# MiloniAtal/gato-python

Measured on AMD Instinct MI355X. Metric: PCG iterations/s, higher is better.
Workload: dtype f64; 1 GPU; iiwa_14_7_k50_f64; STATE_SIZE=14, CONTROL_SIZE=7, KNOT_POINTS=50, max_iters=100, pcg_kernel=resident (one workgroup, mixed 2/1 rows per lane), pcg_workgroups=1, pcg_threads=512

## Files before the change

### gato_python_amd/csrc/gato_assembly.hip

```cpp
#include "gato_common.h"
#include "gato_gj.h"

namespace gato {
namespace {

constexpr int WAVE = 64;

template <typename T, int S, int C>
__global__ void add_rho_kernel(const T *__restrict__ G_in, T rho, T *__restrict__ Gd, size_t n_per_sys, int B)
{
    constexpr int SS = S * S, CC = C * C;
    const size_t total = n_per_sys * B;
    for (size_t i = (size_t)blockIdx.x * blockDim.x + threadIdx.x; i < total; i += (size_t)gridDim.x * blockDim.x) {
        const size_t w = (i % n_per_sys) % (SS + CC);
        const bool diag = w < SS ? (w % (S + 1) == 0) : ((w - SS) % (C + 1) == 0);
        Gd[i] = G_in[i] + (diag ? rho : (T)0);
    }
}

__device__ __forceinline__ void wave_sync() { __syncthreads(); }

template <typename T>
__device__ __forceinline__ void copy_in(T *dst, const T *__restrict__ src, int n, int lane)
{
// ... 221 lines not shown
        Pbd[i] = diag ? (T)1 / Sbd[i] : (T)0;
    }
}

template <typename T, int S>
__global__ __launch_bounds__(WAVE) void ss_kernel(const T *__restrict__ Sbd, T *__restrict__ Pbd, int K, BatchStride bs)
{
    constexpr int SS = S * S;
    int sysi, kidx;
    xcd_knot_map(sysi, kidx);
    Sbd += sysi * bs.bd; Pbd += sysi * bs.bd;
    constexpr bool STAGE = S > 16;
    __shared__ T sT[2][SS];
    __shared__ T stage[STAGE ? 5 * SS : 1];
    const int lane = threadIdx.x;
    for (int k = bs.k_lo + kidx; k < bs.k_hi; k += gridDim.x) {
        T *Pk = Pbd + (size_t)k * 3 * SS;
        const T *sPm = Pk + SS;
        const bool has_l = k > 0, has_r = k < K - 1;
        const T *xl = Sbd + (size_t)k * 3 * SS, *xr = Sbd + (size_t)(k + 1) * 3 * SS;
        const T *pl = Pbd + (size_t)(k - 1) * 3 * SS + SS, *pr = Pbd + (size_t)(k + 1) * 3 * SS + SS;
        wave_sync();
        if constexpr (STAGE) {
            copy_in(stage, sPm, SS, lane);
            if (has_l) { copy_in(stage + SS, xl, SS, lane); copy_in(stage + 2 * SS, pl, SS, lane); }
            if (has_r) { copy_in(stage + 3 * SS, xr, SS, lane); copy_in(stage + 4 * SS, pr, SS, lane); }
            sPm = stage; xl = stage + SS; pl = stage + 2 * SS; xr = stage + 3 * SS; pr = stage + 4 * SS;
            wave_sync();
        }
        if (has_l) {
            const T *sX = xl;
            mfma_for_tiles<T, S, S>(lane,
                [&](int mt, int nt, typename Mfma<T>::acc_t acc) { return mfma_tile<T, S, S, S, false>(sPm, sX, mt, nt, lane, acc); },
                [&](int r, int cc, T v) { sT[0][cc * S + r] = v; });
        }
        if (has_r) {
            const T *sX = xr;
            mfma_for_tiles<T, S, S>(lane,
                [&](int mt, int nt, typename Mfma<T>::acc_t acc) { return mfma_tile<T, S, S, S, true>(sPm, sX, mt, nt, lane, acc); },
                [&](int r, int cc, T v) { sT[1][cc * S + r] = v; });
        }
        wave_sync();
        if (has_l) {
            const T *sPn = pl;
            mfma_for_tiles<T, S, S>(lane,
                [&](int mt, int nt, typename Mfma<T>::acc_t acc) { return mfma_tile<T, S, S, S, false>(sT[0], sPn, mt, nt, lane, acc); },
                [&](int r, int cc, T v) { Pk[cc * S + r] = -v; });
        }
        if (has_r) {
            const T *sPn = pr;
            mfma_for_tiles<T, S, S>(lane,
                [&](int mt, int nt, typename Mfma<T>::acc_t acc) { return mfma_tile<T, S, S, S, false>(sT[1], sPn, mt, nt, lane, acc); },
                [&](int r, int cc, T v) { Pk[2 * SS + cc * S + r] = -v; });
        }
    }
}

template <int NT, typename T>
__device__ __forceinline__ void copy_nt(T *dst, const T *__restrict__ src, int n, int tid)
{
    for (int i = tid; i < n; i += NT) dst[i] = src[i];
}

template <typename T, int M, int N, int NW, typename TileFn, typename StoreFn>
__device__ __forceinline__ void mfma_tiles_on_waves(int wave, int lane, int first, TileFn tile, StoreFn store)
{
    constexpr int NTN = (N + 15) / 16;
#pragma unroll
    for (int mt = 0; mt < (M + 15) / 16; ++mt) {
#pragma unroll
        for (int nt = 0; nt < NTN; ++nt) {
            if ((first + mt * NTN + nt) % NW != wave) continue;
            typename Mfma<T>::acc_t acc = {0, 0, 0, 0};
            acc = tile(mt, nt, acc);
#pragma unroll
            for (int j = 0; j < 4; ++j) {
                const int r = mt * 16 + Mfma<T>::row(lane, j), c = nt * 16 + (lane & 15);
                if (r < M && c < N) store(r, c, acc[j]);
            }
        }
    }
}

template <typename T, int S, int C>
struct AsmLds {
    static constexpr int n = S + C, SS = S * S, CC = C * C, SC = S * C;
    static constexpr int Q = 0;
    static constexpr int R = Q + 3 * SS;
    static constexpr int AB = R + 3 * CC;
    static constexpr int PHI = AB + 2 * (SS + SC);
    static constexpr int BR = PHI + 2 * SS;
    static constexpr int TH = BR + 2 * SC;
    static constexpr int TT = TH + 2 * SS;
    static constexpr int VQ = TT + 2 * SS;
    static constexpr int VV = VQ + 2 * S + C;
    static constexpr int ELEMS = (VV + 3 * S + 3) / 4 * 4;
    static constexpr int PTR_G = 3 * n + 1, PTR_C = 2 * S + 1;
    static constexpr size_t BYTES = sizeof(T) * ELEMS + sizeof(int) * (PTR_G + PTR_C);
};

__device__ __forceinline__ int row_of_entry(const int *ptr, int nrows, int e)
{
    int lo = 0, hi = nrows;
    while (hi - lo > 1) {
        const int mid = (lo + hi) >> 1;
        if (ptr[mid] <= e) lo = mid; else hi = mid;
    }
    return lo;
}

template <typename T, int S, int C, int NT>
__global__ __launch_bounds__(NT, (GatherWaves<T, S>::v)) void gather_kernel(const int *__restrict__ G_row, const int *__restrict__ G_col,
                                                    const T *__restrict__ G_val, const int *__restrict__ C_row,
                                                    const int *__restrict__ C_col, const T *__restrict__ C_val, int K, T rho,
                                                    T *__restrict__ Gd, T *__restrict__ Cd, T *__restrict__ Ginv, BatchStride bs)
{
    constexpr int n = S + C, SS = S * S, CC = C * C, SC = S * C, ABS = SS + SC;
    static_assert(NT % WAVE == 0, "whole waves");
    __shared__ T blk[SS + CC + ABS];
    __shared__ int sPtrG[n + 1], sPtrC[S + 1];
    constexpr int NSLOT = SS + CC + ABS;
    __shared__ unsigned smask[(NSLOT + 31) / 32];
    __shared__ int sown[NSLOT];
    __shared__ int s_coll;
    T *sQ = blk, *sR = blk + SS, *sAB = blk + SS + CC;
    const int tid = threadIdx.x, lane = tid & 63, wave = tid >> 6;
    G_val += blockIdx.y * bs.nnzG; C_val += blockIdx.y * bs.nnzC;
    Gd += blockIdx.y * bs.g; Cd += blockIdx.y * bs.c;
    if (Ginv) Ginv += blockIdx.y * bs.g;
    for (int k = bs.k_lo + blockIdx.x; k < bs.k_hi; k += gridDim.x) {
        const bool last = k == K - 1;
        const int r0 = k * n, nrG = last ? S : n;
        const int c0 = (k + 1) * S, nrC = last ? 0 : S;
        __syncthreads();
        for (int i = tid; i <= nrG; i += NT) sPtrG[i] = G_row[r0 + i];
        if (nrC) for (int i = tid; i <= nrC; i += NT) sPtrC[i] = C_row[c0 + i];
        for (int i = tid; i < SS + CC + ABS; i += NT) blk[i] = (T)0;
        for (int i = tid; i < (NSLOT + 31) / 32; i += NT) smask[i] = 0u;
        if (tid == 0) s_coll = 0;
        __syncthreads();
        const int eG0 = sPtrG[0], nG = sPtrG[nrG] - eG0;
        const int eC0 = nrC ? sPtrC[0] : 0, nC = nrC ? sPtrC[nrC] - eC0 : 0;
        auto slot_of = [&](int t, int colv, T valv, T &v) -> int {
            if (t < nG) {
                const int isr = row_of_entry(sPtrG, nrG, eG0 + t);
                const int isc = colv % n;
                v = valv + (colv == r0 + isr ? rho : (T)0);
                if (isc < S) return isr < S ? isc * S + isr : -1;
                return isr >= S ? SS + (isc - S) * C + (isr - S) : -1;
            }
            const int i = row_of_entry(sPtrC, nrC, eC0 + (t - nG));
            v = valv;
            return colv / n <= k ? SS + CC + (colv % n) * S + i : -1;
        };
        constexpr int U = 4;
        for (int t0 = tid; t0 < nG + nC; t0 += NT * U) {
            int col[U];
            T val[U];
#pragma unroll
            for (int u = 0; u < U; ++u) {
                const int t = t0 + u * NT;
                if (t < nG) { col[u] = G_col[eG0 + t]; val[u] = G_val[eG0 + t]; }
                else if (t < nG + nC) { col[u] = C_col[eC0 + (t - nG)]; val[u] = C_val[eC0 + (t - nG)]; }
            }
#pragma unroll
            for (int u = 0; u < U; ++u) {
                const int t = t0 + u * NT;
                if (t < nG + nC) {
                    T v;
                    const int sl = slot_of(t, col[u], val[u], v);
                    if (sl >= 0) {
                        blk[sl] = v;
                        const unsigned bit = 1u << (sl & 31);
                        if (atomicOr(&smask[sl >> 5], bit) & bit) s_coll = 1;
                    }
                }
            }
        }
        __syncthreads();
        if (s_coll) {
            for (int i = tid; i < NSLOT; i += NT) sown[i] = -1;
            __syncthreads();
            for (int pass = 0; pass < 2; ++pass) {
                for (int t = tid; t < nG + nC; t += NT) {
                    const int colv = t < nG ? G_col[eG0 + t] : C_col[eC0 + (t - nG)];
                    const T valv = t < nG ? G_val[eG0 + t] : C_val[eC0 + (t - nG)];
                    T v;
                    const int sl = slot_of(t, colv, valv, v);
                    if (sl < 0) continue;
                    if (pass == 0) atomicMax(&sown[sl], t);
                    else if (sown[sl] == t) blk[sl] = v;
                }
                __syncthreads();
            }
        }
        __syncthreads();
        const size_t gk = (size_t)k * (SS + CC);
        for (int i = tid; i < SS + (last ? 0 : CC); i += NT) Gd[gk + i] = blk[i];
        if (!last) for (int i = tid; i < ABS; i += NT) Cd[(size_t)k * ABS + i] = sAB[i];
        if (Ginv) {
            if (wave == 0) invert_to<T, S>(sQ, Ginv + gk, lane, (T)1);
            if (wave == (NT > WAVE ? 1 : 0) && !last) invert_to<T, C>(sR, Ginv + gk + SS, lane, (T)1);
        }
    }
}

template <typename T, int S, int C, int NT>
__global__ __launch_bounds__(NT) void assemble_kernel(AsmArgs a, int K, BatchStride bs)
{
    typedef AsmLds<T, S, C> L;
    constexpr int n = S + C, SS = S * S, CC = C * C, SC = S * C, NW = NT / WAVE, ABS = SS + SC;
    static_assert(NW >= 6, "six inversions run side by side");
    constexpr int TILES = ((S + 15) / 16) * ((S + 15) / 16);
    extern __shared__ __align__(16) unsigned char lds_raw[];
    T *lds = (T *)lds_raw;
    T *sQ = lds + L::Q, *sR = lds + L::R, *sAB = lds + L::AB, *sPhi = lds + L::PHI, *sBR = lds + L::BR;
    T *sTh = lds + L::TH, *sT = lds + L::TT, *sq = lds + L::VQ, *sv = lds + L::VV;
    int *sPtrG = (int *)(lds + L::ELEMS), *sPtrC = sPtrG + L::PTR_G;
    constexpr int NSLOT = 3 * SS + 3 * CC + 2 * ABS;
    __shared__ unsigned smask[(NSLOT + 31) / 32];
    __shared__ int sown[NSLOT];
    __shared__ int s_coll;
    const int tid = threadIdx.x, lane = tid & 63, wave = tid >> 6;
    const int sys = blockIdx.y;
    const T *g = (const T *)a.g + sys * bs.n, *c = (const T *)a.c + sys * bs.sk;
    T *Gd = (T *)a.Gd + sys * bs.g, *Cd = (T *)a.Cd + sys * bs.c, *Ginv = (T *)a.Ginv + sys * bs.g;
    T *Sbd = (T *)a.Sbd + sys * bs.bd, *Pbd = (T *)a.Pbd + sys * bs.bd, *gamma = (T *)a.gamma + sys * bs.sk;
    const T rho = (T)a.rho;
    T *const iS = (T *)a.imgS, *const iP = (T *)a.imgP;
    const size_t ild = (size_t)a.img_ld;
    auto imS = [&](int kk, int b, int r, int cc, T v) { if (iS) iS[(size_t)(b * S + cc) * ild + (size_t)kk * S + r] = v; };
    auto imP = [&](int kk, int b, int r, int cc, T v) { if (iP) iP[(size_t)(b * S + cc) * ild + (size_t)kk * S + r] = v; };
    T *sQk = sQ + 2 * SS, *sRk = sR + 2 * CC, *sQm = sQ + SS, *sRm = sR + CC, *sQmm = sQ, *sRmm = sR;
    T *sA1 = sAB + ABS, *sB1 = sA1 + SS, *sA0 = sAB, *sB0 = sAB + SS;
    T *sPhi1 = sPhi + SS, *sPhi0 = sPhi, *sBR1 = sBR + SC, *sBR0 = sBR, *sTh1 = sTh + SS, *sTh0 = sTh;
    int n_stamp = 0;
    auto stamp = [&]() {
        if (a.stamps && blockIdx.x == (K > 2 ? 2 : 0) && sys == 0 && tid == 0) a.stamps[n_stamp++] = __builtin_amdgcn_s_memrealtime();
    };
    stamp();

    for (int k = blockIdx.x; k < K; k += gridDim.x) {
        const bool first = k == 0, last = k == K - 1;
        const bool full0 = k >= 2;
        const size_t gk = (size_t)k * (SS + CC);
        const size_t cm = first ? 0 : (size_t)(k - 1) * ABS;
        T *Sk = Sbd + (size_t)k * 3 * SS, *Pk = Pbd + (size_t)k * 3 * SS;
        __syncthreads();
        if (a.mode == 0) {
            const T *G_val = (const T *)a.G_val + sys * bs.nnzG, *C_val = (const T *)a.C_val + sys * bs.nnzC;
            const int r0 = (k >= 2 ? k - 2 : 0) * n, nrG = k * n + (last ? S : n) - r0;
            const int c0 = (k >= 2 ? k - 1 : 1) * S, nrC = first ? 0 : (k + 1) * S - c0;
            for (int i = tid; i <= nrG; i += NT) sPtrG[i] = a.G_row[r0 + i];
            if (nrC) for (int i = tid; i <= nrC; i += NT) sPtrC[i] = a.C_row[c0 + i];
            for (int i = tid; i < 3 * SS + 3 * CC + 2 * ABS; i += NT) lds[i] = (T)0;
            for (int i = tid; i < (NSLOT + 31) / 32; i += NT) smask[i] = 0u;
            if (tid == 0) s_coll = 0;
            __syncthreads();
            const int eG0 = sPtrG[0], nG = sPtrG[nrG] - eG0;
            const int eC0 = nrC ? sPtrC[0] : 0, nC = nrC ? sPtrC[nrC] - eC0 : 0;
            auto slot_of = [&](int t, int colv, T valv, T &v) -> int {
                if (t < nG) {
                    const int row = r0 + row_of_entry(sPtrG, nrG, eG0 + t);
                    const int knot = row / n, isr = row - knot * n, qi = knot - (k - 2);
                    const int isc = colv % n;
                    v = valv + (colv == row ? rho : (T)0);
                    if (isc < S) return isr < S ? L::Q + qi * SS + isc * S + isr : -1;
                    return isr >= S ? L::R + qi * CC + (isc - S) * C + (isr - S) : -1;
                }
                const int row = c0 + row_of_entry(sPtrC, nrC, eC0 + (t - nG));
                const int br = row / S - 1, i = row - (br + 1) * S;
                v = valv;
                return colv / n <= br ? L::AB + (br - (k - 2)) * ABS + (colv % n) * S + i : -1;
            };
            constexpr int U = 4;
            for (int t0 = tid; t0 < nG + nC; t0 += NT * U) {
                int col[U];
                T val[U];
#pragma unroll
                for (int u = 0; u < U; ++u) {
                    const int t = t0 + u * NT;
                    if (t < nG) { col[u] = a.G_col[eG0 + t]; val[u] = G_val[eG0 + t]; }
                    else if (t < nG + nC) { col[u] = a.C_col[eC0 + (t - nG)]; val[u] = C_val[eC0 + (t - nG)]; }
                }
#pragma unroll
                for (int u = 0; u < U; ++u) {
                    const int t = t0 + u * NT;
                    if (t < nG + nC) {
                        T v;
                        const int sl = slot_of(t, col[u], val[u], v);
                        if (sl >= 0) {
                            lds[sl] = v;
                            const unsigned bit = 1u << (sl & 31);
                            if (atomicOr(&smask[sl >> 5], bit) & bit) s_coll = 1;
                        }
                    }
                }
            }
            __syncthreads();
            if (s_coll) {
                for (int i = tid; i < NSLOT; i += NT) sown[i] = -1;
                __syncthreads();
                for (int pass = 0; pass < 2; ++pass) {
                    for (int t = tid; t < nG + nC; t += NT) {
                        const int colv = t < nG ? a.G_col[eG0 + t] : a.C_col[eC0 + (t - nG)];
                        const T valv = t < nG ? G_val[eG0 + t] : C_val[eC0 + (t - nG)];
                        T v;
                        const int sl = slot_of(t, colv, valv, v);
                        if (sl < 0) continue;
                        if (pass == 0) atomicMax(&sown[sl], t);
                        else if (sown[sl] == t) lds[sl] = v;
                    }
                    __syncthreads();
                }
            }
        } else {
            const T *Gin = a.mode == 2 ? (const T *)a.G_val + sys * bs.g : Gd;
            const T r2 = a.mode == 2 ? rho : (T)0;
#pragma unroll
            for (int qi = 0; qi < 3; ++qi) {
                const int knot = k - 2 + qi;
                if (knot < 0) continue;
                const size_t go = (size_t)knot * (SS + CC);
                for (int i = tid; i < SS; i += NT) sQ[qi * SS + i] = Gin[go + i] + ((i % (S + 1) == 0) ? r2 : (T)0);
                if (knot < K - 1)
                    for (int i = tid; i < CC; i += NT) sR[qi * CC + i] = Gin[go + SS + i] + ((i % (C + 1) == 0) ? r2 : (T)0);
                if (qi < 2 && knot < K - 1) copy_nt<NT>(sAB + qi * ABS, Cd + (size_t)knot * ABS, ABS, tid);
            }
        }
        if (first) { for (int i = tid; i < S; i += NT) sq[i] = g[i]; }
        else {
            copy_nt<NT>(sq, g + (size_t)(k - 1) * n, n, tid);
            for (int i = tid; i < S; i += NT) sq[n + i] = g[(size_t)k * n + i];
        }
        __syncthreads();
        stamp();
        if (a.mode != 1) {
            for (int i = tid; i < SS; i += NT) Gd[gk + i] = sQk[i];
            if (!last) for (int i = tid; i < CC; i += NT) Gd[gk + SS + i] = sRk[i];
            if (a.mode == 0 && !first) for (int i = tid; i < ABS; i += NT) Cd[cm + i] = sA1[i];
        }
        if (first) for (int i = tid; i < SS; i += NT) { Pk[SS + i] = -sQk[i]; imP(0, 1, i % S, i / S, -sQk[i]); }
        if (k == 1) for (int i = tid; i < SS; i += NT) sTh0[i] = -sQm[i];
        __syncthreads();
        if (wave == 0) invert_to<T, S>(sQk, sQk, lane, (T)1);
        else if (wave == 1) { if (!first) invert_to<T, S>(sQm, sQm, lane, (T)1); }
        else if (wave == 2) { if (!first) invert_to<T, C>(sRm, sRm, lane, (T)1); }
        else if (wave == 3) { if (full0) invert_to<T, S>(sQmm, sQmm, lane, (T)1); }
        else if (wave == 4) { if (full0) invert_to<T, C>(sRmm, sRmm, lane, (T)1); }
        else if (wave == 5) { if (!last) invert_to<T, C>(sRk, sRk, lane, (T)1); }
        __syncthreads();
        stamp();
        for (int i = tid; i < SS; i += NT) Ginv[gk + i] = sQk[i];
        if (!last) for (int i = tid; i < CC; i += NT) Ginv[gk + SS + i] = sRk[i];
        if (first) {
            if (wave == 0) mv<T, S, S>(sv, sQk, sq, lane);
            for (int i = tid; i < SS; i += NT) {
                Sk[i] = (T)0;
                Sk[SS + i] = -sQk[i];
                Pk[i] = (T)0;
                if (last) { Pk[2 * SS + i] = (T)0; Sk[2 * SS + i] = (T)0; }
                imS(0, 0, i % S, i / S, (T)0); imS(0, 1, i % S, i / S, -sQk[i]); imP(0, 0, i % S, i / S, (T)0);
                if (last) { imP(0, 2, i % S, i / S, (T)0); imS(0, 2, i % S, i / S, (T)0); }
            }
            __syncthreads();
            for (int i = tid; i < S; i += NT) gamma[i] = c[i] - sv[i];
            continue;
        }
        mfma_tiles_on_waves<T, S, S, NW>(wave, lane, 0,
            [&](int mt, int nt, typename Mfma<T>::acc_t acc) { return mfma_tile<T, S, S, S, false>(sA1, sQm, mt, nt, lane, acc); },
            [&](int r, int cc, T v) {
                sPhi1[cc * S + r] = v;
                Sk[cc * S + r] = -v;
                Sk[2 * SS - 3 * SS + r * S + cc] = -v;
                imS(k, 0, r, cc, -v); imS(k - 1, 2, cc, r, -v);
            });
        mfma_tiles_on_waves<T, S, C, NW>(wave, lane, TILES,
            [&](int mt, int nt, typename Mfma<T>::acc_t acc) { return mfma_tile<T, S, C, C, false>(sB1, sRm, mt, nt, lane, acc); },
            [&](int r, int cc, T v) { sBR1[cc * S + r] = v; });
        if (full0) {
            mfma_tiles_on_waves<T, S, S, NW>(wave, lane, 2 * TILES,
                [&](int mt, int nt, typename Mfma<T>::acc_t acc) { return mfma_tile<T, S, S, S, false>(sA0, sQmm, mt, nt, lane, acc); },
                [&](int r, int cc, T v) { sPhi0[cc * S + r] = v; });
            mfma_tiles_on_waves<T, S, C, NW>(wave, lane, 3 * TILES,
                [&](int mt, int nt, typename Mfma<T>::acc_t acc) { return mfma_tile<T, S, C, C, false>(sB0, sRmm, mt, nt, lane, acc); },
                [&](int r, int cc, T v) { sBR0[cc * S + r] = v; });
        }
        if (wave == NW - 1) mv<T, S, S>(sv, sQk, sq + n, lane);
        __syncthreads();
        if (wave == NW - 1) mv<T, S, S>(sv + S, sPhi1, sq, lane);
        if (wave == NW - 2) mv<T, S, C>(sv + 2 * S, sBR1, sq + S, lane);
        mfma_tiles_on_waves<T, S, S, NW>(wave, lane, 0,
            [&](int mt, int nt, typename Mfma<T>::acc_t acc) {
                acc = mfma_tile<T, S, S, S, true>(sPhi1, sA1, mt, nt, lane, acc);
                return mfma_tile<T, S, C, S, true>(sBR1, sB1, mt, nt, lane, acc);
            },
            [&](int r, int cc, T v) {
                const T th = v + sQk[cc * S + r];
                sTh1[cc * S + r] = th;
                Sk[SS + cc * S + r] = -th;
                imS(k, 1, r, cc, -th);
            });
        if (full0)
            mfma_tiles_on_waves<T, S, S, NW>(wave, lane, TILES,
                [&](int mt, int nt, typename Mfma<T>::acc_t acc) {
                    acc = mfma_tile<T, S, S, S, true>(sPhi0, sA0, mt, nt, lane, acc);
                    return mfma_tile<T, S, C, S, true>(sBR0, sB0, mt, nt, lane, acc);
                },
                [&](int r, int cc, T v) { sTh0[cc * S + r] = v + sQm[cc * S + r]; });
        __syncthreads();
        if (wave == 0) invert_to<T, S>(sTh1, sTh1, lane, (T)-1);
        else if (wave == 1) { if (full0) invert_to<T, S>(sTh0, sTh0, lane, (T)-1); }
        else {
            for (int i = tid - 2 * WAVE; i < S; i += NT - 2 * WAVE) {
                T gt = sv[i] - c[(size_t)k * S + i];
                gt += sv[2 * S + i] + sv[S + i];
                gamma[(size_t)k * S + i] = -gt;
            }
            if (last)
                for (int i = tid - 2 * WAVE; i < SS; i += NT - 2 * WAVE) {
                    Pk[2 * SS + i] = (T)0;
                    Sk[2 * SS + i] = (T)0;
                    imP(k, 2, i % S, i / S, (T)0); imS(k, 2, i % S, i / S, (T)0);
                }
        }
        __syncthreads();
        stamp();
        for (int i = tid; i < SS; i += NT) { Pk[SS + i] = sTh1[i]; imP(k, 1, i % S, i / S, sTh1[i]); }
        mfma_tiles_on_waves<T, S, S, NW>(wave, lane, 0,
            [&](int mt, int nt, typename Mfma<T>::acc_t acc) { return mfma_tile<T, S, S, S, false>(sTh1, sPhi1, mt, nt, lane, acc); },
            [&](int r, int cc, T v) { sT[cc * S + r] = v; });
        mfma_tiles_on_waves<T, S, S, NW>(wave, lane, TILES,
            [&](int mt, int nt, typename Mfma<T>::acc_t acc) { return mfma_tile<T, S, S, S, true>(sTh0, sPhi1, mt, nt, lane, acc); },
            [&](int r, int cc, T v) { sT[SS + cc * S + r] = v; });
        __syncthreads();
        mfma_tiles_on_waves<T, S, S, NW>(wave, lane, 0,
            [&](int mt, int nt, typename Mfma<T>::acc_t acc) { return mfma_tile<T, S, S, S, false>(sT, sTh0, mt, nt, lane, acc); },
            [&](int r, int cc, T v) { Pk[cc * S + r] = v; imP(k, 0, r, cc, v); });
        mfma_tiles_on_waves<T, S, S, NW>(wave, lane, TILES,
            [&](int mt, int nt, typename Mfma<T>::acc_t acc) { return mfma_tile<T, S, S, S, false>(sT + SS, sTh1, mt, nt, lane, acc); },
            [&](int r, int cc, T v) { Pk[2 * SS - 3 * SS + cc * S + r] = v; imP(k - 1, 2, r, cc, v); });
        stamp();
    }
}


template <typename T, int S, int C>
__global__ __launch_bounds__(WAVE) void dz_kernel(const T *__restrict__ Ginv, const T *__restrict__ Cd,
                                                  const T *__restrict__ g, const T *__restrict__ lambda,
                                                  int K, T *__restrict__ dz, BatchStride bs)
{
    constexpr int n = S + C, SS = S * S, CC = C * C, SC = S * C;
    int sysi, kidx;
    xcd_knot_map(sysi, kidx);
    const int msys = bs.rhs > 1 ? sysi / bs.rhs : sysi;
    Ginv += msys * bs.g; Cd += msys * bs.c; g += sysi * bs.n; lambda += sysi * bs.sk;
    dz += sysi * bs.n;
    __shared__ T sQi[SS], sA[SS], sRi[CC > 0 ? CC : 1], sB[SC > 0 ? SC : 1], sl[2 * S], st[S + C], sg[S + C];
    const int lane = threadIdx.x;
    for (int k = bs.k_lo + kidx; k < bs.k_hi; k += gridDim.x) {
        const bool last = k == K - 1;
        wave_sync();
        copy_in(sQi, Ginv + (size_t)k * (SS + CC), SS, lane);
        copy_in(sl, lambda + (size_t)k * S, last ? S : 2 * S, lane);
        copy_in(sg, g + (size_t)k * n, last ? S : n, lane);
        if (!last) {
            copy_in(sRi, Ginv + (size_t)k * (SS + CC) + SS, CC, lane);
            copy_in(sA, Cd + (size_t)k * (SS + SC), SS, lane);
            copy_in(sB, Cd + (size_t)k * (SS + SC) + SS, SC, lane);
        }
        wave_sync();
        if (!last) {
            mTv<T, S, S>(st, sA, sl + S, lane);
            mTv<T, S, C>(st + S, sB, sl + S, lane);
            wave_sync();
            for (int i = lane; i < S; i += WAVE) st[i] = sg[i] - (sl[i] + st[i]);
            for (int i = lane; i < C; i += WAVE) st[S + i] = sg[S + i] - st[S + i];
        } else {
            for (int i = lane; i < S; i += WAVE) st[i] = sg[i] - sl[i];
        }
        wave_sync();
        for (int r = lane; r < S; r += WAVE) {
            T res = (T)0;
#pragma unroll
            for (int cc = 0; cc < S; ++cc) res = gato::fmaT(sQi[r + cc * S], st[cc], res);
            dz[(size_t)k * n + r] = res;
        }
        if (!last) {
            for (int r = lane; r < C; r += WAVE) {
                T res = (T)0;
#pragma unroll
                for (int cc = 0; cc < C; ++cc) res = gato::fmaT(sRi[r + cc * C], st[S + cc], res);
                dz[(size_t)k * n + S + r] = res;
            }
        }
    }
}

}

template <typename T, int S, int C>
int launch_convert(const Dims &d, const int *G_row, const int *G_col, const T *G_val, const int *C_row,
                   const int *C_col, const T *C_val, T rho, T *Gd, T *Cd, T *Ginv, hipStream_t st)
{
    constexpr int NT = S <= 16 ? 64 : 128;
    hipLaunchKernelGGL((gather_kernel<T, S, C, NT>), dim3(d.hi() - d.lo() < (1 << 20) ? d.hi() - d.lo() : (1 << 20), d.B), dim3(NT), 0, st, G_row, G_col,
                       G_val, C_row, C_col, C_val, d.K, rho, Gd, Cd, Ginv, batch_stride(d));
    GATO_HIP_CHECK(hipGetLastError());
    return GATO_OK;
}

template <typename T, int S, int C>
int launch_add_rho(const Dims &d, const T *G_in, T rho, T *Gd, hipStream_t st)
{
    const size_t total = d.g_dense() * d.B;
    const int blocks = (int)((total + 255) / 256 < 2048 ? (total + 255) / 256 : 2048);
    hipLaunchKernelGGL((add_rho_kernel<T, S, C>), dim3(blocks), dim3(256), 0, st, G_in, rho, Gd, d.g_dense(), d.B);
    GATO_HIP_CHECK(hipGetLastError());
    return GATO_OK;
}

static inline int knot_grid(int K) { return K < 8192 ? K : 8192; }

template <typename T, int S, int C>
int launch_form_schur(const Dims &d, const T *Gd, const T *Cd, const T *g, const T *c, T *Sbd, T *Pbd,
// ... 93 lines not shown
```

### gato_python_amd/csrc/gato_capi.hip

```cpp
#include <cmath>
#include <cstdarg>
#include <cstdlib>
#include "gato_solver.h"

namespace gato {

static thread_local char g_err[512] = "";

void set_error(const char *fmt, ...)
{
    va_list ap;
    va_start(ap, fmt);
    vsnprintf(g_err, sizeof(g_err), fmt, ap);
    va_end(ap);
}

}

using namespace gato;

bool solver_usable(const gato_solver *s, const char *entry, const char *unsupported)
{
    if (!s) set_error("%s: null solver", entry);
    else if (s->cl.on || s->cl.local) set_error("%s: the solver is a cluster rank; sharded %s are not supported", entry, unsupported);
// ... 139 lines not shown
    const size_t o_S = take(d.bd() * e * nb), o_P = take(d.bd() * e * nb), o_gam = take(d.sk() * e * nb);
    const size_t o_lam = take(d.sk() * e * nb), o_dz = take(d.N() * e * nb);
    const size_t o_its = take(sizeof(int) * nb);
    const size_t o_vec = take(6 * d.sk() * e);
    const size_t o_part = take((size_t)4 * max_groups * e), o_scal = take(64 * 8), o_done = take(64);
    const size_t o_gh = take((size_t)8 * S * e);
    const size_t o_hist = take(sizeof(double) * (GATO_ETA_HIST_MAX + 1));
    const size_t o_xtab = take(sizeof(void *) * GATO_MAX_RANKS);
    const long long rows = (long long)K * S;
    const bool img = B == 1 && ((s->plan.pair_threads > 0 && rows <= 2ll * s->plan.pair_threads) || (s->plan.mixed_rows > 0 && rows <= s->plan.mixed_rows));
    int img_ld = 0;
    if (img) {
        img_ld = (int)((rows + 63) / 64 * 64) + 128;
        if (img_ld < s->plan.mixed_rows) img_ld = s->plan.mixed_rows;
    }
    const size_t o_iS = take(img ? (size_t)3 * S * img_ld * e : 0), o_iP = take(img ? (size_t)3 * S * img_ld * e : 0);
    s->arena_bytes = off;
    GATO_HIP_CHECK(hipMalloc((void **)&s->arena, off));
    GATO_HIP_CHECK(hipMemset(s->arena, 0, off));
    char *a = s->arena;
    s->slots = (unsigned long long *)(a + o_slots);
    s->status = (int *)(a + o_status);
    s->iters = B > 1 ? (int *)(a + o_its) : (int *)(a + o_status + 8);
    s->final_eta = (double *)(a + o_status + 16);
    s->tune_status = (int *)(a + o_status + 32); s->tune_iters = (int *)(a + o_status + 40); s->tune_eta = (double *)(a + o_status + 48);
    s->dz_flag = (int *)(a + o_status + 56);
    s->G_dense = a + o_G; s->C_dense = a + o_C; s->Ginv = a + o_Gi;
    s->Sbd = a + o_S; s->Pbd = a + o_P; s->gamma = a + o_gam; s->lambda = a + o_lam; s->dz = a + o_dz;
    s->sw.vecs = a + o_vec;
    s->sw.partials = a + o_part; s->sw.scalars = a + o_scal; s->sw.done = (int *)(a + o_done);
    s->sw.max_groups = max_groups;
    s->ghosts = a + o_gh;
    s->eta_hist = (double *)(a + o_hist);
    s->cl_tab = (unsigned long long **)(a + o_xtab);
    if (img) { s->imgS = a + o_iS; s->imgP = a + o_iP; s->img_ld = img_ld; }
    const char *nt = getenv("GATO_NO_TUNE");
    if (!(nt && atoi(nt))) {
        const int rc = gato_solver_tune(s, nullptr);
        if (rc) { gato_solver_destroy(s); return rc; }
    }
    *out = s;
    return GATO_OK;
}

extern "C" int gato_solver_destroy(gato_solver *s)
{
    if (!s) return GATO_OK;
    (void)hipSetDevice(s->device);
    gato_cluster_destroy(s);
    if (s->ev_pcg0) (void)hipEventDestroy(s->ev_pcg0);
    if (s->ev_pcg1) (void)hipEventDestroy(s->ev_pcg1);
    if (s->ev_cal0) (void)hipEventDestroy(s->ev_cal0);
    if (s->ev_cal1) (void)hipEventDestroy(s->ev_cal1);
    for (int i = 0; i < 4; ++i)
        if (s->ev_stage[i]) (void)hipEventDestroy(s->ev_stage[i]);
    if (s->arena) (void)hipFree(s->arena);
    if (s->rhs_ws) (void)hipFree(s->rhs_ws);
    if (s->qp_ws) (void)hipFree(s->qp_ws);
    if (s->pol_ws) (void)hipFree(s->pol_ws);
    if (s->in_arena) (void)hipFree(s->in_arena);
    for (int i = 0; i < 2; ++i)
        if (s->host_ev[i]) (void)hipEventDestroy(s->host_ev[i]);
    if (s->pin) (void)hipHostFree(s->pin);
    delete s;
    return GATO_OK;
}

extern "C" void *gato_solver_buffer(gato_solver *s, int which)
{
    switch (which) {
        case 0: return s->G_dense;
        case 1: return s->C_dense;
        case 2: return s->Ginv;
        case 3: return s->Sbd;
        case 4: return s->Pbd;
        case 5: return s->gamma;
        case 6: return s->lambda;
        case 7: return s->dz;
        case 8: return s->iters;
        case 9: return (unsigned long long *)s->sw.scalars + 8;
        case 10: return s->eta_hist;
        case 11: return s->rhs_ws;
        case 12: return s->qp_pcg_total;
        default: return nullptr;
    }
}

extern "C" int gato_solver_set_option(gato_solver *s, const char *name, int value)
{
    if (!strcmp(name, "pcg_mode")) s->pcg_mode = value;
    else if (!strcmp(name, "pcg_threads")) s->pcg_threads = value;
    else if (!strcmp(name, "pcg_groups")) s->pcg_groups = value;
    else if (!strcmp(name, "asm_mode")) s->asm_mode = value;
    else if (!strcmp(name, "pcg_semi")) s->pcg_semi = value;
    else if (!strcmp(name, "pcg_epoch")) s->pcg_epoch = (unsigned)value;
    else if (!strcmp(name, "cluster_epoch")) s->cl.xepoch = (unsigned)value;
    else if (!strcmp(name, "stamp_asm")) s->stamp_asm = value;
    else if (!strcmp(name, "stamp_pcg")) s->stamp_pcg = value;
    else if (!strcmp(name, "ablate")) s->ablate = value;
    else if (!strcmp(name, "no_single_lds")) s->no_single_lds = value;
    else if (!strcmp(name, "no_pair")) s->no_pair = value;
    else if (!strcmp(name, "wave_pub")) s->wave_pub = value;
    else if (!strcmp(name, "dpp_rows")) s->dpp_rows = value;
    else if (!strcmp(name, "pcg_variant")) s->pcg_variant = value;
    else if (!strcmp(name, "record_eta")) s->record_eta = value;
    else if (!strcmp(name, "xcd_pack")) s->xcd_pack = value;
    else if (!strcmp(name, "xcd_sel")) s->xcd_sel = value < 0 ? -1 : (value & 7);
    else if (!strcmp(name, "true_warm_start")) s->true_warm_start = value;
    else if (!strcmp(name, "timeout_ms")) s->timeout_ms = value > 0 ? value : 2000;
    else if (!strcmp(name, "max_workgroups")) s->max_workgroups = value;
    else if (!strcmp(name, "no_fuse_dz")) s->no_fuse_dz = value;
    else if (!strcmp(name, "no_image")) s->no_image = value;
    else if (!strcmp(name, "coop_launch")) s->coop_launch = value;
    else if (!strcmp(name, "cluster_flat")) s->cluster_flat = value;
    else if (!strcmp(name, "knot_lo") || !strcmp(name, "knot_hi")) {
        if (value < 0 || value > s->d.K) { set_error("%s = %d is outside [0, %d]", name, value, s->d.K); return GATO_EINVAL; }
        (name[5] == 'l' ? s->d.k_lo : s->d.k_hi) = value;
    }
    else if (!strcmp(name, "precon_mode")) {
        if (value < GATO_PRECON_STAIR || value > GATO_PRECON_POINT_JACOBI) { set_error("precon_mode must be 0, 1 or 2"); return GATO_EINVAL; }
        s->precon_mode = value;
    }
    else if (!strcmp(name, "time_stages")) {
        s->time_stages = value;
        if (value && !s->ev_stage[0])
            for (int i = 0; i < 4; ++i) GATO_HIP_CHECK(hipEventCreate(&s->ev_stage[i]));
    }
    else if (!strcmp(name, "batch_nnz_G")) s->d.nnzG = value;
    else if (!strcmp(name, "batch_nnz_C")) s->d.nnzC = value;
    else if (!strcmp(name, "time_pcg")) {
        s->time_pcg = value;
        if (value && !s->ev_pcg0) {
            GATO_HIP_CHECK(hipEventCreate(&s->ev_pcg0));
            GATO_HIP_CHECK(hipEventCreate(&s->ev_pcg1));
        }
    }
    else { set_error("unknown option %s", name); return GATO_EINVAL; }
    return GATO_OK;
}

extern "C" int gato_pcg_last_ms(gato_solver *s, float *ms)
{
    if (!s->time_pcg || !s->ev_pcg0) { set_error("pcg_last_ms: option time_pcg is off"); return GATO_EINVAL; }
    GATO_HIP_CHECK(hipEventSynchronize(s->ev_pcg1));
    GATO_HIP_CHECK(hipEventElapsedTime(ms, s->ev_pcg0, s->ev_pcg1));
    return GATO_OK;
}

extern "C" int gato_last_stage_ms(gato_solver *s, float *ms)
{
    if (!s->time_stages || !s->ev_stage[0]) { set_error("last_stage_ms: option time_stages is off"); return GATO_EINVAL; }
    GATO_HIP_CHECK(hipEventSynchronize(s->ev_stage[3]));
    for (int i = 0; i < 3; ++i) GATO_HIP_CHECK(hipEventElapsedTime(ms + i, s->ev_stage[i], s->ev_stage[i + 1]));
    return GATO_OK;
}

extern "C" int gato_solver_get_option(gato_solver *s, const char *name, int *value)
{
    if (!strcmp(name, "pcg_mode")) *value = s->pcg_mode;
    else if (!strcmp(name, "pcg_threads")) *value = s->pcg_threads;
    else if (!strcmp(name, "pcg_groups")) *value = s->pcg_groups;
    else if (!strcmp(name, "last_groups")) *value = s->last_groups;
    else if (!strcmp(name, "last_threads")) *value = s->last_threads;
    else if (!strcmp(name, "last_mode")) *value = s->last_mode;
    else if (!strcmp(name, "last_pair")) *value = s->last_pair;
    else if (!strcmp(name, "last_dpp")) *value = s->last_dpp;
    else if (!strcmp(name, "last_xcd_sel")) *value = s->last_xcd_sel;
    else if (!strcmp(name, "last_variant")) *value = s->last_variant;
    else if (!strcmp(name, "asm_mode")) *value = s->asm_mode;
    else if (!strcmp(name, "last_asm_fused")) *value = s->last_asm_fused;
    else if (!strcmp(name, "last_image")) *value = s->last_image;
    else if (!strcmp(name, "last_semi")) *value = s->last_semi;
    else if (!strcmp(name, "last_fallback")) *value = s->last_fallback;
    else if (!strcmp(name, "last_dz_fused")) *value = s->dz_fused;
    else if (!strcmp(name, "last_cluster_flat")) *value = s->cl.on ? s->cl.last_flat : 0;
    else if (!strcmp(name, "timeout_ms")) *value = s->timeout_ms;
    else if (!strcmp(name, "precon_mode")) *value = s->precon_mode;
    else if (!strcmp(name, "cluster_mem_kind")) *value = s->cl.on ? s->cl.mem_kind : -1;
    else if (!strcmp(name, "num_cus")) *value = s->num_cus;
    else if (!strcmp(name, "batch")) *value = s->d.B;
    else if (!strcmp(name, "rhs_reserved")) *value = s->rhs_R;
    else if (!strcmp(name, "assembly_valid")) *value = s->as.valid;
    else if (!strcmp(name, "assembly_gen")) *value = (int)s->as.gen;
    else if (!strcmp(name, "true_warm_start")) *value = s->true_warm_start;
    else if (!strcmp(name, "max_semi_knots"))
        *value = s->plan.semi_threads > 0 ? (s->plan.semi_threads / s->d.S + s->plan.semi_rows * s->plan.semi_threads / s->d.S) * (s->num_cus < 256 ? s->num_cus : 256) : 0;
    else if (!strcmp(name, "max_resident_knots")) *value = s->plan.max_knots_per_wg * (s->num_cus < 256 ? s->num_cus : 256);
    else { set_error("unknown option %s", name); return GATO_EINVAL; }
    return GATO_OK;
}

static bool owned(const gato_solver *s, const void *p)
{
    const char *q = (const char *)p;
    return q && ((q >= s->arena && q < s->arena + s->arena_bytes) || (s->rhs_ws && q >= s->rhs_ws && q < s->rhs_ws + s->rhs_ws_bytes));
}
static void note_stage_outputs(gato_solver *s, const void *a, const void *b, const void *c = nullptr, const void *d = nullptr)
{
    if (owned(s, a) || owned(s, b) || owned(s, c) || owned(s, d)) s->as.valid = 0;
}

extern "C" int gato_convert(gato_solver *s, const int *d_G_row, const int *d_G_col, const void *d_G_val,
                            const int *d_C_row, const int *d_C_col, const void *d_C_val, double rho,
                            void *d_G_dense, void *d_C_dense, void *stream)
{
    note_stage_outputs(s, d_G_dense, d_C_dense);
    if (s->d.B > 1 && (s->d.nnzG <= 0 || s->d.nnzC <= 0)) {
        set_error("convert: a batched solver needs the per-system nnz (gato_linsys_device_batched, or options "
                  "batch_nnz_G / batch_nnz_C)");
        return GATO_EINVAL;
    }
    return s->ops->convert(s->d, d_G_row, d_G_col, d_G_val, d_C_row, d_C_col, d_C_val, rho, d_G_dense, d_C_dense,
                           nullptr, (hipStream_t)stream);
}

extern "C" int gato_form_schur(gato_solver *s, const void *d_G_dense, const void *d_C_dense, const void *d_g,
                               const void *d_c, void *d_S, void *d_Pinv, void *d_gamma, void *d_Ginv_dense,
                               void *stream)
{
    note_stage_outputs(s, d_S, d_Pinv, d_gamma, d_Ginv_dense);
    return s->ops->form_schur(s->d, d_G_dense, d_C_dense, d_g, d_c, d_S, d_Pinv, d_gamma, d_Ginv_dense, false,
                              (hipStream_t)stream);
}

extern "C" int gato_form_ss(gato_solver *s, const void *d_S, void *d_Pinv, void *stream)
{
    note_stage_outputs(s, d_Pinv, nullptr);
    return s->ops->form_ss(s->d, d_S, d_Pinv, (hipStream_t)stream);
}

extern "C" int gato_compute_dz(gato_solver *s, const void *d_Ginv_dense, const void *d_C_dense, const void *d_g,
                               const void *d_lambda, void *d_dz, void *stream)
{
    return s->ops->compute_dz(s->d, d_Ginv_dense, d_C_dense, d_g, d_lambda, d_dz, (hipStream_t)stream);
}
```

Measured before the change: 583,800 iterations/s.

## Stage assembly outputs in LDS and batch global write-out at end of knot

Restructures the assemble kernel so the inverses, Schur blocks and preconditioner blocks are kept in dedicated LDS buffers instead of being written to global memory piecemeal inside the MFMA epilogues. All global stores are gathered into one final phase that uses register staging and a per-stream rotation of thread indices. The g and c vector loads are hoisted to the start of each knot, and timestamps are buffered in registers. This reduces scattered stores and barriers during assembly, at the cost of more LDS and more registers. The benchmark metric is PCG iterations per second, so any gain in assembly may not show up in it.

After: 585,900 iterations/s (median of 6 runs). Within noise of the previous version (+0.4%).

```diff
diff --git a/gato_python_amd/csrc/gato_assembly.hip b/gato_python_amd/csrc/gato_assembly.hip
--- a/gato_python_amd/csrc/gato_assembly.hip
+++ b/gato_python_amd/csrc/gato_assembly.hip
@@ -327,6 +327,25 @@
     }
 }
 
+template <int NT, int LEN, typename T, typename F>
+__device__ __forceinline__ void wo_load(T (&v)[(LEN + NT - 1) / NT], int t, int len, F f)
+{
+#pragma unroll
+    for (int u = 0; u < (LEN + NT - 1) / NT; ++u) {
+        const int i = t + u * NT;
+        v[u] = i < len ? f(i) : (T)0;
+    }
+}
+template <int NT, int LEN, typename T, typename F>
+__device__ __forceinline__ void wo_store(const T (&v)[(LEN + NT - 1) / NT], int t, int len, F f)
+{
+#pragma unroll
+    for (int u = 0; u < (LEN + NT - 1) / NT; ++u) {
+        const int i = t + u * NT;
+        if (i < len) f(i, v[u]);
+    }
+}
+
 template <typename T, int S, int C>
 struct AsmLds {
     static constexpr int n = S + C, SS = S * S, CC = C * C, SC = S * C;
@@ -337,9 +356,14 @@
     static constexpr int BR = PHI + 2 * SS;
     static constexpr int TH = BR + 2 * SC;
     static constexpr int TT = TH + 2 * SS;
-    static constexpr int VQ = TT + 2 * SS;
+    static constexpr int GI = TT + 2 * SS;
+    static constexpr int PM = GI + SS + CC;
+    static constexpr int VQ = PM + SS;
     static constexpr int VV = VQ + 2 * S + C;
-    static constexpr int ELEMS = (VV + 3 * S + 3) / 4 * 4;
+    static constexpr int VC = VV + 3 * S;
+    static constexpr int ELEMS = (VC + S + 3) / 4 * 4;
+    static constexpr int PL = PHI, PR = BR;
+    static_assert(2 * SC >= SS, "Pinv[k-1].right is staged over the two BR blocks");
     static constexpr int PTR_G = 3 * n + 1, PTR_C = 2 * S + 1;
     static constexpr size_t BYTES = sizeof(T) * ELEMS + sizeof(int) * (PTR_G + PTR_C);
 };
@@ -456,16 +480,19 @@
     typedef AsmLds<T, S, C> L;
     constexpr int n = S + C, SS = S * S, CC = C * C, SC = S * C, NW = NT / WAVE, ABS = SS + SC;
     static_assert(NW >= 6, "six inversions run side by side");
+    static_assert((NT & (NT - 1)) == 0 && NT >= n + S, "write-out rotation; one thread per hoisted element of g");
     constexpr int TILES = ((S + 15) / 16) * ((S + 15) / 16);
     extern __shared__ __align__(16) unsigned char lds_raw[];
     T *lds = (T *)lds_raw;
     T *sQ = lds + L::Q, *sR = lds + L::R, *sAB = lds + L::AB, *sPhi = lds + L::PHI, *sBR = lds + L::BR;
-    T *sTh = lds + L::TH, *sT = lds + L::TT, *sq = lds + L::VQ, *sv = lds + L::VV;
+    T *sTh = lds + L::TH, *sT = lds + L::TT, *sq = lds + L::VQ, *sv = lds + L::VV, *sc = lds + L::VC;
+    T *sQki = lds + L::GI, *sRki = sQki + SS, *sPm = lds + L::PM, *sPL = lds + L::PL, *sPR = lds + L::PR;
     int *sPtrG = (int *)(lds + L::ELEMS), *sPtrC = sPtrG + L::PTR_G;
     constexpr int NSLOT = 3 * SS + 3 * CC + 2 * ABS;
     __shared__ unsigned smask[(NSLOT + 31) / 32];
     __shared__ int sown[NSLOT];
     __shared__ int s_coll;
+    static_assert(L::BYTES + sizeof(smask) + sizeof(sown) + sizeof(s_coll) <= 160 * 1024, "LDS of one CU");
     const int tid = threadIdx.x, lane = tid & 63, wave = tid >> 6;
     const int sys = blockIdx.y;
     const T *g = (const T *)a.g + sys * bs.n, *c = (const T *)a.c + sys * bs.sk;
@@ -479,11 +506,12 @@
     T *sQk = sQ + 2 * SS, *sRk = sR + 2 * CC, *sQm = sQ + SS, *sRm = sR + CC, *sQmm = sQ, *sRmm = sR;
     T *sA1 = sAB + ABS, *sB1 = sA1 + SS, *sA0 = sAB, *sB0 = sAB + SS;
     T *sPhi1 = sPhi + SS, *sPhi0 = sPhi, *sBR1 = sBR + SC, *sBR0 = sBR, *sTh1 = sTh + SS, *sTh0 = sTh;
+    const bool stamping = a.stamps && blockIdx.x == (K > 2 ? 2 : 0) && sys == 0;
     int n_stamp = 0;
-    auto stamp = [&]() {
-        if (a.stamps && blockIdx.x == (K > 2 ? 2 : 0) && sys == 0 && tid == 0) a.stamps[n_stamp++] = __builtin_amdgcn_s_memrealtime();
-    };
-    stamp();
+    unsigned long long ts[4] = {};
+    auto stamp = [&](int j) { if (stamping) ts[j] = __builtin_amdgcn_s_memrealtime(); };
+    if (stamping && tid == 0) a.stamps[n_stamp] = __builtin_amdgcn_s_memrealtime();
+    ++n_stamp;
 
     for (int k = blockIdx.x; k < K; k += gridDim.x) {
         const bool first = k == 0, last = k == K - 1;
@@ -492,6 +520,10 @@
         const size_t cm = first ? 0 : (size_t)(k - 1) * ABS;
         T *Sk = Sbd + (size_t)k * 3 * SS, *Pk = Pbd + (size_t)k * 3 * SS;
         __syncthreads();
+        __builtin_amdgcn_s_waitcnt(0x0F70);
+        const int nq = first ? S : n + S;
+        const T hq = tid < nq ? g[(first ? (size_t)0 : (size_t)(k - 1) * n) + tid] : (T)0;
+        const T hc = tid < S ? c[(size_t)k * S + tid] : (T)0;
         if (a.mode == 0) {
             const T *G_val = (const T *)a.G_val + sys * bs.nnzG, *C_val = (const T *)a.C_val + sys * bs.nnzC;
             const int r0 = (k >= 2 ? k - 2 : 0) * n, nrG = k * n + (last ? S : n) - r0;
@@ -573,119 +605,122 @@
                 if (qi < 2 && knot < K - 1) copy_nt<NT>(sAB + qi * ABS, Cd + (size_t)knot * ABS, ABS, tid);
             }
         }
-        if (first) { for (int i = tid; i < S; i += NT) sq[i] = g[i]; }
-        else {
-            copy_nt<NT>(sq, g + (size_t)(k - 1) * n, n, tid);
-            for (int i = tid; i < S; i += NT) sq[n + i] = g[(size_t)k * n + i];
-        }
+        if (tid < nq) sq[tid] = hq;
+        if (tid < S) sc[tid] = hc;
+        __builtin_amdgcn_s_waitcnt(0x0F70);
         __syncthreads();
-        stamp();
-        if (a.mode != 1) {
-            for (int i = tid; i < SS; i += NT) Gd[gk + i] = sQk[i];
-            if (!last) for (int i = tid; i < CC; i += NT) Gd[gk + SS + i] = sRk[i];
-            if (a.mode == 0 && !first) for (int i = tid; i < ABS; i += NT) Cd[cm + i] = sA1[i];
-        }
-        if (first) for (int i = tid; i < SS; i += NT) { Pk[SS + i] = -sQk[i]; imP(0, 1, i % S, i / S, -sQk[i]); }
-        if (k == 1) for (int i = tid; i < SS; i += NT) sTh0[i] = -sQm[i];
-        __syncthreads();
-        if (wave == 0) invert_to<T, S>(sQk, sQk, lane, (T)1);
-        else if (wave == 1) { if (!first) invert_to<T, S>(sQm, sQm, lane, (T)1); }
+        stamp(0);
+        if (wave == 0) invert_to<T, S>(sQk, sQki, lane, (T)1);
+        else if (wave == 1) {
+            if (k == 1) for (int i = lane; i < SS; i += WAVE) sTh0[i] = -sQm[i];
+            if (!first) invert_to<T, S>(sQm, sQm, lane, (T)1);
+        }
         else if (wave == 2) { if (!first) invert_to<T, C>(sRm, sRm, lane, (T)1); }
         else if (wave == 3) { if (full0) invert_to<T, S>(sQmm, sQmm, lane, (T)1); }
         else if (wave == 4) { if (full0) invert_to<T, C>(sRmm, sRmm, lane, (T)1); }
-        else if (wave == 5) { if (!last) invert_to<T, C>(sRk, sRk, lane, (T)1); }
+        else if (wave == 5) { if (!last) invert_to<T, C>(sRk, sRki, lane, (T)1); }
         __syncthreads();
-        stamp();
-        for (int i = tid; i < SS; i += NT) Ginv[gk + i] = sQk[i];
-        if (!last) for (int i = tid; i < CC; i += NT) Ginv[gk + SS + i] = sRk[i];
+        stamp(1);
         if (first) {
-            if (wave == 0) mv<T, S, S>(sv, sQk, sq, lane);
-            for (int i = tid; i < SS; i += NT) {
-                Sk[i] = (T)0;
-                Sk[SS + i] = -sQk[i];
-                Pk[i] = (T)0;
-                if (last) { Pk[2 * SS + i] = (T)0; Sk[2 * SS + i] = (T)0; }
-                imS(0, 0, i % S, i / S, (T)0); imS(0, 1, i % S, i / S, -sQk[i]); imP(0, 0, i % S, i / S, (T)0);
-                if (last) { imP(0, 2, i % S, i / S, (T)0); imS(0, 2, i % S, i / S, (T)0); }
-            }
+            if (wave == 0) mv<T, S, S>(sv, sQki, sq, lane);
+        } else {
+            mfma_tiles_on_waves<T, S, S, NW>(wave, lane, 0,
+                [&](int mt, int nt, typename Mfma<T>::acc_t acc) { return mfma_tile<T, S, S, S, false>(sA1, sQm, mt, nt, lane, acc); },
+                [&](int r, int cc, T v) { sPhi1[cc * S + r] = v; });
+            mfma_tiles_on_waves<T, S, C, NW>(wave, lane, TILES,
+                [&](int mt, int nt, typename Mfma<T>::acc_t acc) { return mfma_tile<T, S, C, C, false>(sB1, sRm, mt, nt, lane, acc); },
+                [&](int r, int cc, T v) { sBR1[cc * S + r] = v; });
+            if (full0) {
+                mfma_tiles_on_waves<T, S, S, NW>(wave, lane, 2 * TILES,
+                    [&](int mt, int nt, typename Mfma<T>::acc_t acc) { return mfma_tile<T, S, S, S, false>(sA0, sQmm, mt, nt, lane, acc); },
+                    [&](int r, int cc, T v) { sPhi0[cc * S + r] = v; });
+                mfma_tiles_on_waves<T, S, C, NW>(wave, lane, 3 * TILES,
+                    [&](int mt, int nt, typename Mfma<T>::acc_t acc) { return mfma_tile<T, S, C, C, false>(sB0, sRmm, mt, nt, lane, acc); },
+                    [&](int r, int cc, T v) { sBR0[cc * S + r] = v; });
+            }
+            if (wave == NW - 1) mv<T, S, S>(sv, sQki, sq + n, lane);
             __syncthreads();
-            for (int i = tid; i < S; i += NT) gamma[i] = c[i] - sv[i];
-            continue;
-        }
-        mfma_tiles_on_waves<T, S, S, NW>(wave, lane, 0,
-            [&](int mt, int nt, typename Mfma<T>::acc_t acc) { return mfma_tile<T, S, S, S, false>(sA1, sQm, mt, nt, lane, acc); },
-            [&](int r, int cc, T v) {
-                sPhi1[cc * S + r] = v;
-                Sk[cc * S + r] = -v;
-                Sk[2 * SS - 3 * SS + r * S + cc] = -v;
-                imS(k, 0, r, cc, -v); imS(k - 1, 2, cc, r, -v);
+            if (wave == NW - 1) mv<T, S, S>(sv + S, sPhi1, sq, lane);
+            if (wave == NW - 2) mv<T, S, C>(sv + 2 * S, sBR1, sq + S, lane);
+            mfma_tiles_on_waves<T, S, S, NW>(wave, lane, 0,
+                [&](int mt, int nt, typename Mfma<T>::acc_t acc) {
+                    acc = mfma_tile<T, S, S, S, true>(sPhi1, sA1, mt, nt, lane, acc);
+                    return mfma_tile<T, S, C, S, true>(sBR1, sB1, mt, nt, lane, acc);
+                },
+                [&](int r, int cc, T v) { sTh1[cc * S + r] = v + sQki[cc * S + r]; });
+            if (full0)
+                mfma_tiles_on_waves<T, S, S, NW>(wave, lane, TILES,
+                    [&](int mt, int nt, typename Mfma<T>::acc_t acc) {
+                        acc = mfma_tile<T, S, S, S, true>(sPhi0, sA0, mt, nt, lane, acc);
+                        return mfma_tile<T, S, C, S, true>(sBR0, sB0, mt, nt, lane, acc);
+                    },
+                    [&](int r, int cc, T v) { sTh0[cc * S + r] = v + sQm[cc * S + r]; });
+            __syncthreads();
+            if (wave == 0) invert_to<T, S>(sTh1, sPm, lane, (T)-1);
+            else if (wave == 1) { if (full0) invert_to<T, S>(sTh0, sTh0, lane, (T)-1); }
+            __syncthreads();
+            stamp(2);
+            mfma_tiles_on_waves<T, S, S, NW>(wave, lane, 0,
+                [&](int mt, int nt, typename Mfma<T>::acc_t acc) { return mfma_tile<T, S, S, S, false>(sPm, sPhi1, mt, nt, lane, acc); },
+                [&](int r, int cc, T v) { sT[cc * S + r] = v; });
+            mfma_tiles_on_waves<T, S, S, NW>(wave, lane, TILES,
+                [&](int mt, int nt, typename Mfma<T>::acc_t acc) { return mfma_tile<T, S, S, S, true>(sTh0, sPhi1, mt, nt, lane, acc); },
+                [&](int r, int cc, T v) { sT[SS + cc * S + r] = v; });
+            __syncthreads();
+            mfma_tiles_on_waves<T, S, S, NW>(wave, lane, 0,
+                [&](int mt, int nt, typename Mfma<T>::acc_t acc) { return mfma_tile<T, S, S, S, false>(sT, sTh0, mt, nt, lane, acc); },
+                [&](int r, int cc, T v) { sPL[cc * S + r] = v; });
+            mfma_tiles_on_waves<T, S, S, NW>(wave, lane, TILES,
+                [&](int mt, int nt, typename Mfma<T>::acc_t acc) { return mfma_tile<T, S, S, S, false>(sT + SS, sPm, mt, nt, lane, acc); },
+                [&](int r, int cc, T v) { sPR[cc * S + r] = v; });
+        }
+        __syncthreads();
+        {
+            const int glen = last ? SS : SS + CC;
+            const bool wG = a.mode != 1, wC = a.mode == 0 && !first;
+            auto rot = [&](int s) { return (tid + NT * SS - s * SS) & (NT - 1); };
+            constexpr int UG = (SS + CC + NT - 1) / NT, UC = (ABS + NT - 1) / NT, UB = (SS + NT - 1) / NT, UV = (S + NT - 1) / NT;
+            T wGd[UG], wCd[UC], wGi[UG], wSl[UB], wSm[UB], wSr[UB], wPl[UB], wPm[UB], wPr[UB], wga[UV];
+            if (wG) wo_load<NT, SS + CC>(wGd, rot(0), glen, [&](int i) { return i < SS ? sQk[i] : sRk[i - SS]; });
+            if (wC) wo_load<NT, ABS>(wCd, rot(1), ABS, [&](int i) { return sA1[i]; });
+            wo_load<NT, SS + CC>(wGi, rot(2), glen, [&](int i) { return sQki[i]; });
+            wo_load<NT, SS>(wSl, rot(3), SS, [&](int i) { return first ? (T)0 : -sPhi1[i]; });
+            wo_load<NT, SS>(wSm, rot(4), SS, [&](int i) { return first ? -sQki[i] : -sTh1[i]; });
+            wo_load<NT, SS>(wPl, rot(5), SS, [&](int i) { return first ? (T)0 : sPL[i]; });
+            wo_load<NT, SS>(wPm, rot(6), SS, [&](int i) { return first ? -sQk[i] : sPm[i]; });
+            if (!first) {
+                wo_load<NT, SS>(wSr, rot(7), SS, [&](int i) { return -sPhi1[(i % S) * S + i / S]; });
+                wo_load<NT, SS>(wPr, rot(8), SS, [&](int i) { return sPR[i]; });
+            }
+            wo_load<NT, S>(wga, rot(9), S, [&](int i) {
+                if (first) return sc[i] - sv[i];
+                T gt = sv[i] - sc[i];
+                gt += sv[2 * S + i] + sv[S + i];
+                return -gt;
             });
-        mfma_tiles_on_waves<T, S, C, NW>(wave, lane, TILES,
-            [&](int mt, int nt, typename Mfma<T>::acc_t acc) { return mfma_tile<T, S, C, C, false>(sB1, sRm, mt, nt, lane, acc); },
-            [&](int r, int cc, T v) { sBR1[cc * S + r] = v; });
-        if (full0) {
-            mfma_tiles_on_waves<T, S, S, NW>(wave, lane, 2 * TILES,
-                [&](int mt, int nt, typename Mfma<T>::acc_t acc) { return mfma_tile<T, S, S, S, false>(sA0, sQmm, mt, nt, lane, acc); },
-                [&](int r, int cc, T v) { sPhi0[cc * S + r] = v; });
-            mfma_tiles_on_waves<T, S, C, NW>(wave, lane, 3 * TILES,
-                [&](int mt, int nt, typename Mfma<T>::acc_t acc) { return mfma_tile<T, S, C, C, false>(sB0, sRmm, mt, nt, lane, acc); },
-                [&](int r, int cc, T v) { sBR0[cc * S + r] = v; });
-        }
-        if (wave == NW - 1) mv<T, S, S>(sv, sQk, sq + n, lane);
-        __syncthreads();
-        if (wave == NW - 1) mv<T, S, S>(sv + S, sPhi1, sq, lane);
-        if (wave == NW - 2) mv<T, S, C>(sv + 2 * S, sBR1, sq + S, lane);
-        mfma_tiles_on_waves<T, S, S, NW>(wave, lane, 0,
-            [&](int mt, int nt, typename Mfma<T>::acc_t acc) {
-                acc = mfma_tile<T, S, S, S, true>(sPhi1, sA1, mt, nt, lane, acc);
-                return mfma_tile<T, S, C, S, true>(sBR1, sB1, mt, nt, lane, acc);
-            },
-            [&](int r, int cc, T v) {
-                const T th = v + sQk[cc * S + r];
-                sTh1[cc * S + r] = th;
-                Sk[SS + cc * S + r] = -th;
-                imS(k, 1, r, cc, -th);
-            });
-        if (full0)
-            mfma_tiles_on_waves<T, S, S, NW>(wave, lane, TILES,
-                [&](int mt, int nt, typename Mfma<T>::acc_t acc) {
-                    acc = mfma_tile<T, S, S, S, true>(sPhi0, sA0, mt, nt, lane, acc);
-                    return mfma_tile<T, S, C, S, true>(sBR0, sB0, mt, nt, lane, acc);
-                },
-                [&](int r, int cc, T v) { sTh0[cc * S + r] = v + sQm[cc * S + r]; });
-        __syncthreads();
-        if (wave == 0) invert_to<T, S>(sTh1, sTh1, lane, (T)-1);
-        else if (wave == 1) { if (full0) invert_to<T, S>(sTh0, sTh0, lane, (T)-1); }
-        else {
-            for (int i = tid - 2 * WAVE; i < S; i += NT - 2 * WAVE) {
-                T gt = sv[i] - c[(size_t)k * S + i];
-                gt += sv[2 * S + i] + sv[S + i];
-                gamma[(size_t)k * S + i] = -gt;
-            }
+            if (wG) wo_store<NT, SS + CC>(wGd, rot(0), glen, [&](int i, T v) { Gd[gk + i] = v; });
+            if (wC) wo_store<NT, ABS>(wCd, rot(1), ABS, [&](int i, T v) { Cd[cm + i] = v; });
+            wo_store<NT, SS + CC>(wGi, rot(2), glen, [&](int i, T v) { Ginv[gk + i] = v; });
+            wo_store<NT, SS>(wSl, rot(3), SS, [&](int i, T v) { Sk[i] = v; imS(k, 0, i % S, i / S, v); });
+            wo_store<NT, SS>(wSm, rot(4), SS, [&](int i, T v) { Sk[SS + i] = v; imS(k, 1, i % S, i / S, v); });
+            wo_store<NT, SS>(wPl, rot(5), SS, [&](int i, T v) { Pk[i] = v; imP(k, 0, i % S, i / S, v); });
+            wo_store<NT, SS>(wPm, rot(6), SS, [&](int i, T v) { Pk[SS + i] = v; imP(k, 1, i % S, i / S, v); });
+            if (!first) {
+                wo_store<NT, SS>(wSr, rot(7), SS, [&](int i, T v) { Sk[i - SS] = v; imS(k - 1, 2, i % S, i / S, v); });
+                wo_store<NT, SS>(wPr, rot(8), SS, [&](int i, T v) { Pk[i - SS] = v; imP(k - 1, 2, i % S, i / S, v); });
+            }
+            wo_store<NT, S>(wga, rot(9), S, [&](int i, T v) { gamma[(size_t)k * S + i] = v; });
             if (last)
-                for (int i = tid - 2 * WAVE; i < SS; i += NT - 2 * WAVE) {
+                for (int i = rot(10); i < SS; i += NT) {
                     Pk[2 * SS + i] = (T)0;
                     Sk[2 * SS + i] = (T)0;
                     imP(k, 2, i % S, i / S, (T)0); imS(k, 2, i % S, i / S, (T)0);
                 }
         }
-        __syncthreads();
-        stamp();
-        for (int i = tid; i < SS; i += NT) { Pk[SS + i] = sTh1[i]; imP(k, 1, i % S, i / S, sTh1[i]); }
-        mfma_tiles_on_waves<T, S, S, NW>(wave, lane, 0,
-            [&](int mt, int nt, typename Mfma<T>::acc_t acc) { return mfma_tile<T, S, S, S, false>(sTh1, sPhi1, mt, nt, lane, acc); },
-            [&](int r, int cc, T v) { sT[cc * S + r] = v; });
-        mfma_tiles_on_waves<T, S, S, NW>(wave, lane, TILES,
-            [&](int mt, int nt, typename Mfma<T>::acc_t acc) { return mfma_tile<T, S, S, S, true>(sTh0, sPhi1, mt, nt, lane, acc); },
-            [&](int r, int cc, T v) { sT[SS + cc * S + r] = v; });
-        __syncthreads();
-        mfma_tiles_on_waves<T, S, S, NW>(wave, lane, 0,
-            [&](int mt, int nt, typename Mfma<T>::acc_t acc) { return mfma_tile<T, S, S, S, false>(sT, sTh0, mt, nt, lane, acc); },
-            [&](int r, int cc, T v) { Pk[cc * S + r] = v; imP(k, 0, r, cc, v); });
-        mfma_tiles_on_waves<T, S, S, NW>(wave, lane, TILES,
-            [&](int mt, int nt, typename Mfma<T>::acc_t acc) { return mfma_tile<T, S, S, S, false>(sT + SS, sTh1, mt, nt, lane, acc); },
-            [&](int r, int cc, T v) { Pk[2 * SS - 3 * SS + cc * S + r] = v; imP(k - 1, 2, r, cc, v); });
-        stamp();
+        stamp(3);
+        if (stamping && tid == 0 && n_stamp + 4 <= 16)
+            for (int j = 0; j < 4; ++j) a.stamps[n_stamp + j] = ts[j];
+        n_stamp += 4;
     }
 }
 
diff --git a/gato_python_amd/csrc/gato_capi.hip b/gato_python_amd/csrc/gato_capi.hip
--- a/gato_python_amd/csrc/gato_capi.hip
+++ b/gato_python_amd/csrc/gato_capi.hip
@@ -245,6 +245,8 @@
         case 10: return s->eta_hist;
         case 11: return s->rhs_ws;
         case 12: return s->qp_pcg_total;
+        case 13: return s->imgS;
+        case 14: return s->imgP;
         default: return nullptr;
     }
 }
@@ -333,6 +335,7 @@
     else if (!strcmp(name, "asm_mode")) *value = s->asm_mode;
     else if (!strcmp(name, "last_asm_fused")) *value = s->last_asm_fused;
     else if (!strcmp(name, "last_image")) *value = s->last_image;
+    else if (!strcmp(name, "img_ld")) *value = s->imgS ? s->img_ld : 0;
     else if (!strcmp(name, "last_semi")) *value = s->last_semi;
     else if (!strcmp(name, "last_fallback")) *value = s->last_fallback;
     else if (!strcmp(name, "last_dz_fused")) *value = s->dz_fused;
```
